# xhuan8/SoccerPlayerShapePose

Hardware: NVIDIA B200
Metric: SMPL meshes/sec fwd+bwd (higher is better)
Workload: dtype f32 (bf16x3 split on tcgen05, fp32 accumulate)

## Files before the change

### soccerplayershapepose_b200/csrc/lbs.cu

```cuda
#include "lbs_tiles.cuh"

namespace b200smpl {


struct CtaRange {
  int begin, end;
};
__device__ __forceinline__ CtaRange make_cta_range(int ngroups, int nitems) {
  const long long total = (long long)ngroups * nitems;
  CtaRange r;
  r.begin = (int)(total * blockIdx.x / gridDim.x);
  r.end = (int)(total * (blockIdx.x + 1) / gridDim.x);
  return r;
}

template <int HV>
__device__ __forceinline__ void issue_item(float4* vbuf, uint32_t* stash, uint64_t* bar, const float4* __restrict__ vp_group,
                                           const uint32_t* __restrict__ vplan, int t) {
  using SH = ItemShape<HV>;
  mbar_expect_tx(bar, SH::TX_BYTES);
  bulk_g2s(vbuf, vp_group + (size_t)t * (SH::NCH4 * 32), SH::VP_WORDS * 4, bar);
  bulk_g2s(stash, vplan + (size_t)t * SH::PLAN_WORDS, SH::PLAN_WORDS * 4, bar);
}
template <int HV>
__device__ __forceinline__ void global_to_tile_scalar(float* tile, const float* src0, size_t row_stride, int nrows,
                                                      int ncols, int lane) {
  for (int r = 0; r < 32; ++r)
    for (int c = lane; c < ItemShape<HV>::ROWS; c += 32)
      tile[r * ItemShape<HV>::HROW + c] = (r < nrows && c < ncols) ? src0[(size_t)r * row_stride + c] : 0.f;
}

constexpr int FWD_RUN = 1;
constexpr int FWD_HV = 16;
constexpr int FWD_WARPS = 8;
constexpr int FWD_THREADS = FWD_WARPS * 32;
constexpr int FWD_WARP_WORDS = ItemShape<FWD_HV>::TILE_WORDS + 2 * (ItemShape<FWD_HV>::VP_WORDS + ItemShape<FWD_HV>::PLAN_WORDS) + 4;
constexpr size_t FWD_SMEM = (size_t)(AG_WORDS + FWD_WARPS * FWD_WARP_WORDS) * 4 + 16;

template <bool HI>
__device__ __forceinline__ void load_slot2(SlotXY& s, SlotZ2& z, const float* A_s, int joint, int lane) {
  const float4* p = reinterpret_cast<const float4*>(A_s) + joint * 96 + lane;
  const float4 q0 = p[0], q1 = p[32], q2 = p[64];
  s.c0 = mk2(q0.x, q0.y); s.c1 = mk2(q0.z, q0.w); s.c2 = mk2(q1.x, q1.y); s.t = mk2(q1.z, q1.w);
  z.r20 = set_half<HI>(z.r20, q2.x); z.r21 = set_half<HI>(z.r21, q2.y);
  z.r22 = set_half<HI>(z.r22, q2.z); z.t2 = set_half<HI>(z.t2, q2.w);
}

__device__ __forceinline__ void skin_fwd4(Slots& s, const float* A_s, int lane, const uint32_t* meta_s,
                                          const float4* wts_s, uint32_t force, float tx, float ty, float tz,
                                          const float4* vp_s, float* row_out) {
  const uint4 m4 = *reinterpret_cast<const uint4*>(meta_s);
  const uint32_t mts[4] = {m4.x | force, m4.y, m4.z, m4.w};
  float4 ws[4];
#pragma unroll
  for (int i = 0; i < 4; ++i) ws[i] = wts_s[i];
  float P[12], o[12];
#pragma unroll
  for (int i = 0; i < 3; ++i) {
    const float4 v = vp_s[i * 32];
    P[i * 4] = v.x; P[i * 4 + 1] = v.y; P[i * 4 + 2] = v.z; P[i * 4 + 3] = v.w;
  }
  const f2 txy = mk2(tx, ty), tz0 = mk2(tz, 0.f);
#pragma unroll
  for (int i = 0; i < 4; ++i) {
    const uint32_t mt = mts[i];
    const float4 w = ws[i];
    if (mt & (0xFu << 20)) {
      if (mt & (1u << 20)) load_slot2<false>(s.s0, s.zA, A_s, mt & 31, lane);
      if (mt & (1u << 21)) load_slot2<true>(s.s1, s.zA, A_s, (mt >> 5) & 31, lane);
      if (mt & (1u << 22)) load_slot2<false>(s.s2, s.zB, A_s, (mt >> 10) & 31, lane);
      if (mt & (1u << 23)) load_slot2<true>(s.s3, s.zB, A_s, (mt >> 15) & 31, lane);
    }
    const f2 px = bc2(P[i * 3]), py = bc2(P[i * 3 + 1]), pz = bc2(P[i * 3 + 2]);
    f2 oxy = txy;
#define B200_SKIN_XY(sl, wk) oxy = fma2(bc2(wk), fma2(sl.c0, px, fma2(sl.c1, py, fma2(sl.c2, pz, sl.t))), oxy);
    B200_SKIN_XY(s.s0, w.x)
    B200_SKIN_XY(s.s1, w.y)
    B200_SKIN_XY(s.s2, w.z)
    B200_SKIN_XY(s.s3, w.w)
#undef B200_SKIN_XY
    f2 oz = fma2(mk2(w.x, w.y), fma2(s.zA.r20, px, fma2(s.zA.r21, py, fma2(s.zA.r22, pz, s.zA.t2))), tz0);
    oz = fma2(mk2(w.z, w.w), fma2(s.zB.r20, px, fma2(s.zB.r21, py, fma2(s.zB.r22, pz, s.zB.t2))), oz);
    o[i * 3] = lo2(oxy); o[i * 3 + 1] = hi2(oxy); o[i * 3 + 2] = lo2(oz) + hi2(oz);
  }
#pragma unroll
  for (int i = 0; i < 3; ++i)
    *reinterpret_cast<float4*>(row_out + i * 4) = make_float4(o[i * 4], o[i * 4 + 1], o[i * 4 + 2], o[i * 4 + 3]);
}

__global__ void __launch_bounds__(FWD_THREADS, 1)
lbs_fwd_kernel(const float4* __restrict__ vpB, int nc4, const float4* __restrict__ A_blk, int b0, int nb, int ngroups,
               const float* __restrict__ transl, float* __restrict__ verts, int V, int nitems, int vec_ok,
               const uint32_t* __restrict__ vplan) {
  constexpr int HV = FWD_HV;
  using SH = ItemShape<HV>;
  extern __shared__ __align__(128) float smem[];
  const int warp = threadIdx.x >> 5, lane = threadIdx.x & 31;
  float* A_s = smem;
  float* wbase = smem + AG_WORDS + warp * FWD_WARP_WORDS;
  float* tile = wbase;
  float4* vbufs = reinterpret_cast<float4*>(wbase + SH::TILE_WORDS);
  uint32_t* stash = reinterpret_cast<uint32_t*>(wbase + SH::TILE_WORDS + 2 * SH::VP_WORDS);
  uint64_t* wbar = reinterpret_cast<uint64_t*>(wbase + SH::TILE_WORDS + 2 * (SH::VP_WORDS + SH::PLAN_WORDS));
  uint64_t* bar = reinterpret_cast<uint64_t*>(smem + AG_WORDS + FWD_WARPS * FWD_WARP_WORDS);
  if (lane == 0) {
    mbar_init(&wbar[0], 1);
    mbar_init(&wbar[1], 1);
    if (warp == 0) mbar_init(bar, 1);
    asm volatile("fence.mbarrier_init.release.cluster;" ::: "memory");
  }
  __syncthreads();
  pdl_wait();
  if (threadIdx.x == 0) pdl_trigger();
  uint32_t a_phase = 0, n_used = 0;
  const CtaRange cta = make_cta_range(ngroups, nitems);
  for (int seg0 = cta.begin; seg0 < cta.end;) {
    const int g = seg0 / nitems;
    if (threadIdx.x == 0) {
      mbar_expect_tx(bar, AG_WORDS * 4);
      bulk_g2s(A_s, A_blk + (size_t)g * (AG_WORDS / 4), AG_WORDS * 4, bar);
    }
    const int seg1 = min(cta.end, (g + 1) * nitems);
    const int len = seg1 - seg0;
    const int sb = seg0 - g * nitems;
    auto off_at = [&](int n) { const int r = n / FWD_RUN; return (r * FWD_WARPS + warp) * FWD_RUN + (n - r * FWD_RUN); };
    if (off_at(0) < len) {
      const float4* vp_g = vpB + (size_t)g * nc4 * 32;
      float tx = 0.f, ty = 0.f, tz = 0.f;
      if (transl != nullptr && g * 32 + lane < nb) {
        const float* tp = transl + (size_t)(b0 + g * 32 + lane) * 3;
        tx = tp[0]; ty = tp[1]; tz = tp[2];
      }
      const int nrows = min(32, nb - g * 32);
      float* v_g = verts + (size_t)(b0 + g * 32) * V * 3;
      float* my_row = tile + lane * SH::HROW;
      if (lane == 0) {
        const uint32_t b = n_used & 1;
        issue_item<HV>(vbufs + b * (SH::NCH4 * 32), stash + b * SH::PLAN_WORDS, &wbar[b], vp_g, vplan, sb + off_at(0));
      }
      Slots sl;
      sl.zA.r20 = sl.zA.r21 = sl.zA.r22 = sl.zA.t2 = sl.zB.r20 = sl.zB.r21 = sl.zB.r22 = sl.zB.t2 = mk2(0.f, 0.f);
      mbar_wait(bar, a_phase);
      for (int n = 0;; ++n) {
        const int t = sb + off_at(n);
        if (t >= sb + len) break;
        const int tn = sb + off_at(n + 1);
        const uint32_t b = n_used & 1;
        if (tn < sb + len && lane == 0)
          issue_item<HV>(vbufs + (b ^ 1) * (SH::NCH4 * 32), stash + (b ^ 1) * SH::PLAN_WORDS, &wbar[b ^ 1], vp_g, vplan, tn);
        mbar_wait(&wbar[b], (n_used >> 1) & 1);
        const float4* vp_s = vbufs + b * (SH::NCH4 * 32) + lane;
        const uint32_t* st = stash + b * SH::PLAN_WORDS;
#pragma unroll 1
        for (int u = 0; u < HV / 4; ++u)
          skin_fwd4(sl, A_s, lane, plan_meta(st, u), plan_wts(st, u), (u == 0 && n % FWD_RUN == 0) ? (0xFu << 20) : 0u,
                    tx, ty, tz, vp_s + u * 96, my_row + u * 12);
        __syncwarp();
        {
          const int vbase = t * HV;
          const int ncols = max(0, min(HV, V - vbase)) * 3;
          float* dst0 = v_g + (size_t)vbase * 3;
          if (!vec_ok) tile_to_global_scalar<HV>(tile, dst0, (size_t)V * 3, nrows, ncols, lane);
          else tile_to_global<HV>(tile, dst0, (size_t)V * 3, nrows, ncols, lane);
        }
        __syncwarp();
        ++n_used;
      }
    }
    seg0 = seg1;
    a_phase ^= 1;
    if (seg0 < cta.end) __syncthreads();
  }
}

constexpr int BWD_HV = 8;
constexpr int BWD_WARPS = 8;
constexpr int BWD_THREADS = BWD_WARPS * 32;
constexpr int BWD_NTILE = 2;
constexpr int BWD_WARP_WORDS = BWD_NTILE * ItemShape<BWD_HV>::TILE_WORDS + 2 * (ItemShape<BWD_HV>::VP_WORDS + ItemShape<BWD_HV>::PLAN_WORDS) + 4;
constexpr size_t BWD_SMEM = (size_t)(AG_WORDS + BWD_WARPS * BWD_WARP_WORDS) * 4 + 16;

template <bool HI>
__device__ __forceinline__ void load_rot_half(SlotPair& P, const float* A_s, int joint, int lane) {
  const float4* p = reinterpret_cast<const float4*>(A_s) + joint * 96 + lane;
  const float4 q0 = p[0], q1 = p[32], q2 = p[64];
  P.R[0] = set_half<HI>(P.R[0], q0.x); P.R[3] = set_half<HI>(P.R[3], q0.y);
  P.R[1] = set_half<HI>(P.R[1], q0.z); P.R[4] = set_half<HI>(P.R[4], q0.w);
  P.R[2] = set_half<HI>(P.R[2], q1.x); P.R[5] = set_half<HI>(P.R[5], q1.y);
  P.R[6] = set_half<HI>(P.R[6], q2.x); P.R[7] = set_half<HI>(P.R[7], q2.y); P.R[8] = set_half<HI>(P.R[8], q2.z);
}

__device__ __forceinline__ void skin_bwd4(BwdState& s, const float* A_s, float* __restrict__ dA_g,
                                          int lane, const uint32_t* meta_s, const float4* wts_s, uint32_t force,
                                          const float4* vp_s, float* row_io) {
  const uint4 m4 = *reinterpret_cast<const uint4*>(meta_s);
  const uint32_t mts[4] = {m4.x | force, m4.y, m4.z, m4.w};
  float P[12], G[12];
#pragma unroll
  for (int i = 0; i < 3; ++i) {
    const float4 v = vp_s[i * 32];
    P[i * 4] = v.x; P[i * 4 + 1] = v.y; P[i * 4 + 2] = v.z; P[i * 4 + 3] = v.w;
    const float4 h = *reinterpret_cast<const float4*>(row_io + i * 4);
    G[i * 4] = h.x; G[i * 4 + 1] = h.y; G[i * 4 + 2] = h.z; G[i * 4 + 3] = h.w;
  }
  float4 w = wts_s[0];
#pragma unroll
  for (int i = 0; i < 4; ++i) {
    const uint32_t mt = mts[i];
    const float4 wn = wts_s[i < 3 ? i + 1 : 3];
    if (mt & (0xFu << 20)) {
      const uint32_t pv = s.prev;
      if (mt & (1u << 20)) { flush_half<false>(s.A, dA_g, pv & 31, lane); load_rot_half<false>(s.A, A_s, mt & 31, lane); }
      if (mt & (1u << 21)) { flush_half<true>(s.A, dA_g, (pv >> 5) & 31, lane); load_rot_half<true>(s.A, A_s, (mt >> 5) & 31, lane); }
      if (mt & (1u << 22)) { flush_half<false>(s.B, dA_g, (pv >> 10) & 31, lane); load_rot_half<false>(s.B, A_s, (mt >> 10) & 31, lane); }
      if (mt & (1u << 23)) { flush_half<true>(s.B, dA_g, (pv >> 15) & 31, lane); load_rot_half<true>(s.B, A_s, (mt >> 15) & 31, lane); }
    }
    s.prev = mt;
    const f2 px = bc2(P[i * 3]), py = bc2(P[i * 3 + 1]), pz = bc2(P[i * 3 + 2]);
    const float gx = G[i * 3], gy = G[i * 3 + 1], gz = G[i * 3 + 2];
    s.sx += gx; s.sy += gy; s.sz += gz;
    const f2 wA = mk2(w.x, w.y), wB = mk2(w.z, w.w);
    const f2 hxA = mul2(wA, bc2(gx)), hyA = mul2(wA, bc2(gy)), hzA = mul2(wA, bc2(gz));
    const f2 hxB = mul2(wB, bc2(gx)), hyB = mul2(wB, bc2(gy)), hzB = mul2(wB, bc2(gz));
    f2 qx = fma2(s.A.R[0], hxA, fma2(s.A.R[3], hyA, mul2(s.A.R[6], hzA)));
    f2 qy = fma2(s.A.R[1], hxA, fma2(s.A.R[4], hyA, mul2(s.A.R[7], hzA)));
    f2 qz = fma2(s.A.R[2], hxA, fma2(s.A.R[5], hyA, mul2(s.A.R[8], hzA)));
    qx = fma2(s.B.R[0], hxB, fma2(s.B.R[3], hyB, fma2(s.B.R[6], hzB, qx)));
    qy = fma2(s.B.R[1], hxB, fma2(s.B.R[4], hyB, fma2(s.B.R[7], hzB, qy)));
    qz = fma2(s.B.R[2], hxB, fma2(s.B.R[5], hyB, fma2(s.B.R[8], hzB, qz)));
    G[i * 3] = lo2(qx) + hi2(qx); G[i * 3 + 1] = lo2(qy) + hi2(qy); G[i * 3 + 2] = lo2(qz) + hi2(qz);
#define B200_ACC(P_, hx_, hy_, hz_)                                                                  \
  P_.D[0] = fma2(hx_, px, P_.D[0]); P_.D[1] = fma2(hx_, py, P_.D[1]); P_.D[2] = fma2(hx_, pz, P_.D[2]);   \
  P_.D[3] = add2(P_.D[3], hx_);                                                                      \
  P_.D[4] = fma2(hy_, px, P_.D[4]); P_.D[5] = fma2(hy_, py, P_.D[5]); P_.D[6] = fma2(hy_, pz, P_.D[6]);   \
  P_.D[7] = add2(P_.D[7], hy_);                                                                      \
  P_.D[8] = fma2(hz_, px, P_.D[8]); P_.D[9] = fma2(hz_, py, P_.D[9]); P_.D[10] = fma2(hz_, pz, P_.D[10]); \
  P_.D[11] = add2(P_.D[11], hz_);
    B200_ACC(s.A, hxA, hyA, hzA)
    B200_ACC(s.B, hxB, hyB, hzB)
#undef B200_ACC
    w = wn;
  }
#pragma unroll
  for (int i = 0; i < 3; ++i)
    *reinterpret_cast<float4*>(row_io + i * 4) = make_float4(G[i * 4], G[i * 4 + 1], G[i * 4 + 2], G[i * 4 + 3]);
}

__global__ void __launch_bounds__(BWD_THREADS, 1)
lbs_bwd_kernel(const float4* __restrict__ vpB, int nc4, const float4* __restrict__ A_blk, int b0, int nb, int ngroups,
               const float* __restrict__ grad_verts, int V, int nitems, int vec_ok,
               const uint32_t* __restrict__ vplan,
               __nv_bfloat16* __restrict__ dvp_hi, __nv_bfloat16* __restrict__ dvp_lo,
               float* __restrict__ dA_acc, float* __restrict__ dtr_acc) {
  constexpr int HV = BWD_HV;
  using SH = ItemShape<HV>;
  extern __shared__ __align__(128) float smem[];
  const int warp = threadIdx.x >> 5, lane = threadIdx.x & 31;
  float* A_s = smem;
  float* wbase = smem + AG_WORDS + warp * BWD_WARP_WORDS;
  float* tiles = wbase;
  float4* vbufs = reinterpret_cast<float4*>(wbase + BWD_NTILE * SH::TILE_WORDS);
  uint32_t* stash = reinterpret_cast<uint32_t*>(wbase + BWD_NTILE * SH::TILE_WORDS + 2 * SH::VP_WORDS);
  uint64_t* wbar = reinterpret_cast<uint64_t*>(wbase + BWD_NTILE * SH::TILE_WORDS + 2 * (SH::VP_WORDS + SH::PLAN_WORDS));
  uint64_t* bar = reinterpret_cast<uint64_t*>(smem + AG_WORDS + BWD_WARPS * BWD_WARP_WORDS);
  if (lane == 0) {
    mbar_init(&wbar[0], 1);
    mbar_init(&wbar[1], 1);
    if (warp == 0) mbar_init(bar, 1);
    asm volatile("fence.mbarrier_init.release.cluster;" ::: "memory");
  }
  __syncthreads();
  if (threadIdx.x == 0) pdl_trigger();
  uint32_t a_phase = 0, n_used = 0;
  const size_t row_stride = (size_t)V * 3;
  const CtaRange cta = make_cta_range(ngroups, nitems);
  for (int seg0 = cta.begin; seg0 < cta.end;) {
    const int g = seg0 / nitems;
    if (threadIdx.x == 0) {
      mbar_expect_tx(bar, AG_WORDS * 4);
      bulk_g2s(A_s, A_blk + (size_t)g * (AG_WORDS / 4), AG_WORDS * 4, bar);
    }
    const int seg1 = min(cta.end, (g + 1) * nitems);
    const int len = seg1 - seg0;
    const int it0 = seg0 - g * nitems + len * warp / BWD_WARPS;
    const int it1 = seg0 - g * nitems + len * (warp + 1) / BWD_WARPS;
    if (it0 < it1) {
      float* dA_g = dA_acc + (size_t)g * AG_WORDS;
      const float4* vp_g = vpB + (size_t)g * nc4 * 32;
      const float* dv_g = grad_verts + (size_t)(b0 + g * 32) * V * 3;
      const int nrows = max(0, min(32, nb - g * 32));
      if (lane == 0) {
        const uint32_t b = n_used & 1;
        issue_item<HV>(vbufs + b * (SH::NCH4 * 32), stash + b * SH::PLAN_WORDS, &wbar[b], vp_g, vplan, it0);
      }
      int tb = 0;
      if (vec_ok) issue_rows<HV>(tiles, dv_g + (size_t)it0 * HV * 3, row_stride, nrows, max(0, min(HV, V - it0 * HV)) * 3, lane);
      cp_async_commit();
      if (!vec_ok)
        global_to_tile_scalar<HV>(tiles, dv_g + (size_t)it0 * HV * 3, row_stride, nrows, max(0, min(HV, V - it0 * HV)) * 3, lane);
      BwdState st;
#pragma unroll
      for (int e = 0; e < AELEMS; ++e) st.A.D[e] = st.B.D[e] = mk2(0.f, 0.f);
#pragma unroll
      for (int e = 0; e < 9; ++e) st.A.R[e] = st.B.R[e] = mk2(0.f, 0.f);
      st.prev = 0u;
      st.sx = st.sy = st.sz = 0.f;
      __syncwarp();
      mbar_wait(bar, a_phase);
      for (int t = it0; t < it1; ++t) {
        const bool more = t + 1 < it1;
        const uint32_t b = n_used & 1;
        float* tile = tiles + tb * SH::TILE_WORDS;
        float* my_row = tile + lane * SH::HROW;
        if (more) {
          if (lane == 0)
            issue_item<HV>(vbufs + (b ^ 1) * (SH::NCH4 * 32), stash + (b ^ 1) * SH::PLAN_WORDS, &wbar[b ^ 1], vp_g, vplan, t + 1);
          if (vec_ok)
            issue_rows<HV>(tiles + (tb ^ 1) * SH::TILE_WORDS, dv_g + (size_t)(t + 1) * HV * 3, row_stride, nrows,
                           max(0, min(HV, V - (t + 1) * HV)) * 3, lane);
        }
        cp_async_commit();
        cp_async_wait<1>();
        __syncwarp();
        mbar_wait(&wbar[b], (n_used >> 1) & 1);
        const float4* vp_s = vbufs + b * (SH::NCH4 * 32) + lane;
        const uint32_t* ps = stash + b * SH::PLAN_WORDS;
#pragma unroll 1
        for (int u = 0; u < HV / 4; ++u)
          skin_bwd4(st, A_s, dA_g, lane, plan_meta(ps, u), plan_wts(ps, u), (u == 0 && t == it0) ? (0xFu << 20) : 0u,
                    vp_s + u * 96, my_row + u * 12);
        {
          const size_t o0 = (((size_t)(g >> 2) * (nc4 >> 1) + t * SH::NCH8) * 128 + (g & 3) * 32 + lane) * 8;
#pragma unroll
          for (int c = 0; c < SH::NCH8; ++c) {
            const float4 x = *reinterpret_cast<const float4*>(my_row + c * 8);
            const float4 y = *reinterpret_cast<const float4*>(my_row + c * 8 + 4);
            const float ch[8] = {x.x, x.y, x.z, x.w, y.x, y.y, y.z, y.w};
            store_dvp_chunk(ch, dvp_hi + o0 + c * 1024, dvp_lo ? dvp_lo + o0 + c * 1024 : nullptr);
          }
        }
        __syncwarp();
        if (more && !vec_ok)
          global_to_tile_scalar<HV>(tiles + (tb ^ 1) * SH::TILE_WORDS, dv_g + (size_t)(t + 1) * HV * 3, row_stride, nrows,
                                    max(0, min(HV, V - (t + 1) * HV)) * 3, lane);
        tb ^= 1;
        __syncwarp();
        ++n_used;
      }
      bwd_close_group(st, dA_g, dtr_acc + (size_t)g * 96, lane);
    }
    seg0 = seg1;
    a_phase ^= 1;
    if (seg0 < cta.end) __syncthreads();
  }
}

static int run_grid(int ngroups, int nitems, int warps, int num_sms) {
  const long long total = (long long)ngroups * nitems;
  return (int)std::max<long long>(1, std::min<long long>(num_sms, (total + warps - 1) / warps));
}

int launch_lbs_fwd(const DevModel& m, const float* vpB, int S, const float* A_blk, int b0, int nb,
                   const float* transl, float* verts, int num_sms, cudaStream_t st) {
  if (nb <= 0) return 0;
  const int groups = (nb + 31) / 32;
  const int nitems = m.ntiles * (TILE_V / FWD_HV);
  const int vec_ok = ((m.V & 1) == 0 && (reinterpret_cast<uintptr_t>(verts) & 7) == 0) ? 1 : 0;
  B200_SMEM_ATTR_ONCE(lbs_fwd_kernel, FWD_SMEM);
  LaunchTimer _timer("lbs_fwd", st);
  B200_CUDA_TRY(launch_k(lbs_fwd_kernel, dim3(run_grid(groups, nitems, FWD_WARPS, num_sms)), dim3(FWD_THREADS), FWD_SMEM, st, true,
                         reinterpret_cast<const float4*>(vpB), m.n_pad / 4, reinterpret_cast<const float4*>(A_blk), b0, nb, groups,
                         transl, verts, m.V, nitems, vec_ok, m.vplan));
  B200_LAUNCH_CHECK("lbs_fwd");
  return 0;
}

int launch_lbs_bwd(const DevModel& m, const float* vpB, int S, int Sw, const float* A_blk, int b0, int nb,
                   const float* grad_verts, __nv_bfloat16* dvp_hi, __nv_bfloat16* dvp_lo, float* dA_acc,
                   float* dtr_acc, int num_sms, cudaStream_t st) {
  const int groups = Sw / 32;
  const int nitems = m.ntiles * (TILE_V / BWD_HV);
  const int vec_ok = ((m.V & 1) == 0 && (reinterpret_cast<uintptr_t>(grad_verts) & 7) == 0) ? 1 : 0;
  B200_SMEM_ATTR_ONCE(lbs_bwd_kernel, BWD_SMEM);
  LaunchTimer _timer("lbs_bwd", st);
  lbs_bwd_kernel<<<run_grid(groups, nitems, BWD_WARPS, num_sms), BWD_THREADS, BWD_SMEM, st>>>(
      reinterpret_cast<const float4*>(vpB), m.n_pad / 4, reinterpret_cast<const float4*>(A_blk), b0, nb, groups, grad_verts, m.V,
      nitems, vec_ok, m.vplan, dvp_hi, dvp_lo, dA_acc, dtr_acc);
  B200_LAUNCH_CHECK("lbs_bwd");
  return 0;
}

}
```

### soccerplayershapepose_b200/csrc/lbs_tiles.cuh

```cuda
#pragma once

#include "skin_common.cuh"

namespace b200smpl {

template <int HV>
struct ItemShape {
  static constexpr int ROWS = HV * 3;
  static constexpr int HROW = ROWS + 4;
  static constexpr int TILE_WORDS = 32 * HROW;
  static constexpr int NCH4 = ROWS / 4;
  static constexpr int NCH8 = ROWS / 8;
  static constexpr int PAIRS = ROWS / 2;
  static constexpr int VP_WORDS = NCH4 * 128;
  static constexpr int PLAN_WORDS = (HV / 8) * 40;
  static constexpr uint32_t TX_BYTES = (VP_WORDS + PLAN_WORDS) * 4;
  static_assert((HROW / 4) % 2 == 1 && ROWS % 8 == 0 && HV % 8 == 0, "item shape");
};

__device__ __forceinline__ const float4* plan_wts(const uint32_t* stash, int u) {
  return reinterpret_cast<const float4*>(stash + (u >> 1) * 40 + (u & 1) * 16);
}
__device__ __forceinline__ const uint32_t* plan_meta(const uint32_t* stash, int u) {
  return stash + (u >> 1) * 40 + 32 + (u & 1) * 4;
}

template <int HV>
__device__ __forceinline__ void tile_to_global_full(const float* tile, float* dst0, size_t row_stride, int lane) {
  using SH = ItemShape<HV>;
  constexpr int RPP = 96 / SH::PAIRS, J = 32 / RPP;
  float* gp[3];
  const float* sp[3];
#pragma unroll
  for (int kk = 0; kk < 3; ++kk) {
    const int piece = kk * 32 + lane, rr = piece / SH::PAIRS, c = (piece - rr * SH::PAIRS) * 2;
    gp[kk] = dst0 + (size_t)rr * row_stride + c;
    sp[kk] = tile + rr * SH::HROW + c;
  }
  const size_t step = (size_t)RPP * row_stride;
#pragma unroll
  for (int j = 0; j < J; ++j)
#pragma unroll
    for (int kk = 0; kk < 3; ++kk) {
      st_stream2(gp[kk], *reinterpret_cast<const float2*>(sp[kk] + j * RPP * SH::HROW));
      gp[kk] += step;
    }
}
template <int HV>
__device__ __forceinline__ void tile_to_global(const float* tile, float* dst0, size_t row_stride, int nrows,
                                               int ncols, int lane) {
  using SH = ItemShape<HV>;
  if (nrows == 32 && ncols == SH::ROWS) {
    tile_to_global_full<HV>(tile, dst0, row_stride, lane);
    return;
  }
#pragma unroll 1
  for (int k = 0; k < SH::PAIRS; ++k) {
    const int piece = k * 32 + lane;
    const int r = piece / SH::PAIRS;
    const int c = (piece - r * SH::PAIRS) * 2;
    const float2 v = *reinterpret_cast<const float2*>(tile + r * SH::HROW + c);
    float* dst = dst0 + (size_t)r * row_stride + c;
    if (r < nrows) {
      if (c + 1 < ncols) st_stream2(dst, v);
      else if (c < ncols) st_stream(dst, v.x);
    }
  }
}

template <int HV>
__device__ __forceinline__ void tile_to_global_scalar(const float* tile, float* dst0, size_t row_stride, int nrows,
                                                      int ncols, int lane) {
  for (int r = 0; r < nrows; ++r)
    for (int c = lane; c < ncols; c += 32) dst0[(size_t)r * row_stride + c] = tile[r * ItemShape<HV>::HROW + c];
}

struct SlotXY {
  f2 c0, c1, c2, t;
};
struct SlotZ2 {
  f2 r20, r21, r22, t2;
};
struct Slots {
  SlotXY s0, s1, s2, s3;
  SlotZ2 zA, zB;
};

__device__ __forceinline__ void cp_async8_zfill(void* dst_smem, const void* src, int src_bytes) {
  asm volatile("cp.async.ca.shared.global.L2::256B [%0], [%1], 8, %2;" ::"r"(smem_addr(dst_smem)), "l"(src), "r"(src_bytes)
               : "memory");
}
__device__ __forceinline__ void cp_async_commit() { asm volatile("cp.async.commit_group;" ::: "memory"); }
template <int N>
__device__ __forceinline__ void cp_async_wait() { asm volatile("cp.async.wait_group %0;" ::"n"(N) : "memory"); }
template <int HV>
__device__ __forceinline__ void issue_rows(float* tile, const float* __restrict__ src0, size_t row_stride, int nrows,
                                           int ncols, int lane) {
  using SH = ItemShape<HV>;
  constexpr int RPP = 96 / SH::PAIRS, J = 32 / RPP;
  if (nrows == 32 && ncols == SH::ROWS) {
    const float* gp[3];
    float* sp[3];
#pragma unroll
    for (int kk = 0; kk < 3; ++kk) {
      const int piece = kk * 32 + lane, rr = piece / SH::PAIRS, c = (piece - rr * SH::PAIRS) * 2;
      gp[kk] = src0 + (size_t)rr * row_stride + c;
      sp[kk] = tile + rr * SH::HROW + c;
    }
    const size_t step = (size_t)RPP * row_stride;
#pragma unroll
    for (int j = 0; j < J; ++j)
#pragma unroll
      for (int kk = 0; kk < 3; ++kk) {
        cp_async8_zfill(sp[kk] + j * RPP * SH::HROW, gp[kk], 8);
        gp[kk] += step;
      }
    return;
  }
#pragma unroll 1
  for (int k = 0; k < SH::PAIRS; ++k) {
    const int piece = k * 32 + lane;
    const int r = piece / SH::PAIRS;
    const int c = (piece - r * SH::PAIRS) * 2;
    const bool ok = r < nrows && c < ncols;
    const int bytes = ok ? (c + 1 < ncols ? 8 : 4) : 0;
    cp_async8_zfill(tile + r * SH::HROW + c, ok ? src0 + (size_t)r * row_stride + c : src0, bytes);
  }
}

struct SlotPair {
  f2 R[9];
  f2 D[AELEMS];
};
struct BwdState {
  SlotPair A, B;
  uint32_t prev;
  float sx, sy, sz;
};
template <bool HI>
__device__ __forceinline__ void flush_half(SlotPair& P, float* dA_g, int joint, int lane) {
  float* p = dA_g + (size_t)joint * AELEMS * 32 + lane;
#pragma unroll
  for (int e = 0; e < AELEMS; ++e) {
    red_add(p + e * 32, get_half<HI>(P.D[e]));
    P.D[e] = set_half<HI>(P.D[e], 0.f);
  }
}

__device__ __forceinline__ void bwd_close_group(BwdState& s, float* dA_g, float* dtr_g, int lane) {
  flush_half<false>(s.A, dA_g, s.prev & 31, lane);
  flush_half<true>(s.A, dA_g, (s.prev >> 5) & 31, lane);
  flush_half<false>(s.B, dA_g, (s.prev >> 10) & 31, lane);
  flush_half<true>(s.B, dA_g, (s.prev >> 15) & 31, lane);
  red_add(dtr_g + lane, s.sx);
  red_add(dtr_g + 32 + lane, s.sy);
  red_add(dtr_g + 64 + lane, s.sz);
  s.sx = s.sy = s.sz = 0.f;
}


}
```

Baseline: 6.948 million.

## Pipeline backward skinning loads in three stages with cp.async mbarrier completion

The backward LBS kernel goes from a double-buffered scheme, which used separate cp.async commit/wait groups and bulk-copy mbarriers, to a three-stage ring. Each stage's mbarrier tracks both the bulk vertex and plan copies and the per-lane 16-byte cp.async gradient-row copies via cp.async.mbarrier.arrive. Gradient rows are now fetched as aligned 16-byte chunks regardless of alignment, and each lane reads at a per-row phase offset, so the scalar fallback path and the vec_ok flag are removed. The intent is deeper prefetch and fewer warp syncs and wait stalls. The costs are more shared memory per warp and over-fetching at row boundaries.

Measured after the change: 6.325 million, median of 6. -9.0%, worse.

```diff
diff --git a/soccerplayershapepose_b200/csrc/lbs.cu b/soccerplayershapepose_b200/csrc/lbs.cu
--- a/soccerplayershapepose_b200/csrc/lbs.cu
+++ b/soccerplayershapepose_b200/csrc/lbs.cu
@@ -21,13 +21,6 @@
   mbar_expect_tx(bar, SH::TX_BYTES);
   bulk_g2s(vbuf, vp_group + (size_t)t * (SH::NCH4 * 32), SH::VP_WORDS * 4, bar);
   bulk_g2s(stash, vplan + (size_t)t * SH::PLAN_WORDS, SH::PLAN_WORDS * 4, bar);
-}
-template <int HV>
-__device__ __forceinline__ void global_to_tile_scalar(float* tile, const float* src0, size_t row_stride, int nrows,
-                                                      int ncols, int lane) {
-  for (int r = 0; r < 32; ++r)
-    for (int c = lane; c < ItemShape<HV>::ROWS; c += 32)
-      tile[r * ItemShape<HV>::HROW + c] = (r < nrows && c < ncols) ? src0[(size_t)r * row_stride + c] : 0.f;
 }
 
 constexpr int FWD_RUN = 1;
@@ -176,9 +169,41 @@
 constexpr int BWD_HV = 8;
 constexpr int BWD_WARPS = 8;
 constexpr int BWD_THREADS = BWD_WARPS * 32;
-constexpr int BWD_NTILE = 2;
-constexpr int BWD_WARP_WORDS = BWD_NTILE * ItemShape<BWD_HV>::TILE_WORDS + 2 * (ItemShape<BWD_HV>::VP_WORDS + ItemShape<BWD_HV>::PLAN_WORDS) + 4;
+constexpr int BWD_STAGES = 3;
+constexpr int BWD_STAGE_WORDS = ItemShape<BWD_HV>::TILE_WORDS + ItemShape<BWD_HV>::VP_WORDS + ItemShape<BWD_HV>::PLAN_WORDS;
+constexpr int BWD_BAR_WORDS = (2 * BWD_STAGES + 3) / 4 * 4;
+constexpr int BWD_WARP_WORDS = BWD_STAGES * BWD_STAGE_WORDS + BWD_BAR_WORDS;
 constexpr size_t BWD_SMEM = (size_t)(AG_WORDS + BWD_WARPS * BWD_WARP_WORDS) * 4 + 16;
+static_assert(BWD_SMEM <= 227 * 1024, "lbs_bwd shared memory");
+static_assert(BWD_STAGE_WORDS % 4 == 0 && BWD_WARP_WORDS % 4 == 0, "16-byte aligned staging buffers");
+
+template <int HV>
+__device__ __forceinline__ void issue_bwd_item(float* tile, float4* vbuf, uint32_t* stash, uint64_t* bar,
+                                               const float4* __restrict__ vp_group, const uint32_t* __restrict__ vplan,
+                                               const float* dv_g, size_t row_stride, int nrows, int ncols, int t,
+                                               int lane) {
+  using SH = ItemShape<HV>;
+  constexpr int GR = SH::HROW / 4;
+  if (lane == 0) {
+    mbar_expect_tx(bar, SH::TX_BYTES);
+    bulk_g2s(vbuf, vp_group + (size_t)t * (SH::NCH4 * 32), SH::VP_WORDS * 4, bar);
+    bulk_g2s(stash, vplan + (size_t)t * SH::PLAN_WORDS, SH::PLAN_WORDS * 4, bar);
+  }
+  if (ncols > 0) {
+#pragma unroll
+    for (int k = 0; k < GR; ++k) {
+      const int piece = k * 32 + lane, r = piece / GR, q = piece - r * GR;
+      if (r < nrows) {
+        const uintptr_t a = reinterpret_cast<uintptr_t>(dv_g + (size_t)r * row_stride + (size_t)t * SH::ROWS);
+        const uintptr_t w0 = a & ~(uintptr_t)15;
+        if (w0 + 16 * q < a + (uintptr_t)ncols * 4)
+          asm volatile("cp.async.cg.shared.global [%0], [%1], 16;" ::"r"(smem_addr(tile + r * SH::HROW + 4 * q)),
+                       "l"(w0 + 16 * q) : "memory");
+      }
+    }
+  }
+  asm volatile("cp.async.mbarrier.arrive.noinc.shared::cta.b64 [%0];" ::"r"(smem_addr(bar)) : "memory");
+}
 
 template <bool HI>
 __device__ __forceinline__ void load_rot_half(SlotPair& P, const float* A_s, int joint, int lane) {
@@ -192,7 +217,7 @@
 
 __device__ __forceinline__ void skin_bwd4(BwdState& s, const float* A_s, float* __restrict__ dA_g,
                                           int lane, const uint32_t* meta_s, const float4* wts_s, uint32_t force,
-                                          const float4* vp_s, float* row_io) {
+                                          const float4* vp_s, const float* row_in, float* row_out) {
   const uint4 m4 = *reinterpret_cast<const uint4*>(meta_s);
   const uint32_t mts[4] = {m4.x | force, m4.y, m4.z, m4.w};
   float P[12], G[12];
@@ -200,9 +225,9 @@
   for (int i = 0; i < 3; ++i) {
     const float4 v = vp_s[i * 32];
     P[i * 4] = v.x; P[i * 4 + 1] = v.y; P[i * 4 + 2] = v.z; P[i * 4 + 3] = v.w;
-    const float4 h = *reinterpret_cast<const float4*>(row_io + i * 4);
-    G[i * 4] = h.x; G[i * 4 + 1] = h.y; G[i * 4 + 2] = h.z; G[i * 4 + 3] = h.w;
-  }
+  }
+#pragma unroll
+  for (int i = 0; i < 12; ++i) G[i] = row_in[i];
   float4 w = wts_s[0];
 #pragma unroll
   for (int i = 0; i < 4; ++i) {
@@ -243,12 +268,12 @@
   }
 #pragma unroll
   for (int i = 0; i < 3; ++i)
-    *reinterpret_cast<float4*>(row_io + i * 4) = make_float4(G[i * 4], G[i * 4 + 1], G[i * 4 + 2], G[i * 4 + 3]);
+    *reinterpret_cast<float4*>(row_out + i * 4) = make_float4(G[i * 4], G[i * 4 + 1], G[i * 4 + 2], G[i * 4 + 3]);
 }
 
 __global__ void __launch_bounds__(BWD_THREADS, 1)
 lbs_bwd_kernel(const float4* __restrict__ vpB, int nc4, const float4* __restrict__ A_blk, int b0, int nb, int ngroups,
-               const float* __restrict__ grad_verts, int V, int nitems, int vec_ok,
+               const float* __restrict__ grad_verts, int V, int nitems,
                const uint32_t* __restrict__ vplan,
                __nv_bfloat16* __restrict__ dvp_hi, __nv_bfloat16* __restrict__ dvp_lo,
                float* __restrict__ dA_acc, float* __restrict__ dtr_acc) {
@@ -259,13 +284,13 @@
   float* A_s = smem;
   float* wbase = smem + AG_WORDS + warp * BWD_WARP_WORDS;
   float* tiles = wbase;
-  float4* vbufs = reinterpret_cast<float4*>(wbase + BWD_NTILE * SH::TILE_WORDS);
-  uint32_t* stash = reinterpret_cast<uint32_t*>(wbase + BWD_NTILE * SH::TILE_WORDS + 2 * SH::VP_WORDS);
-  uint64_t* wbar = reinterpret_cast<uint64_t*>(wbase + BWD_NTILE * SH::TILE_WORDS + 2 * (SH::VP_WORDS + SH::PLAN_WORDS));
+  float4* vbufs = reinterpret_cast<float4*>(wbase + BWD_STAGES * SH::TILE_WORDS);
+  uint32_t* stash = reinterpret_cast<uint32_t*>(wbase + BWD_STAGES * (SH::TILE_WORDS + SH::VP_WORDS));
+  uint64_t* wbar = reinterpret_cast<uint64_t*>(wbase + BWD_STAGES * BWD_STAGE_WORDS);
   uint64_t* bar = reinterpret_cast<uint64_t*>(smem + AG_WORDS + BWD_WARPS * BWD_WARP_WORDS);
   if (lane == 0) {
-    mbar_init(&wbar[0], 1);
-    mbar_init(&wbar[1], 1);
+#pragma unroll
+    for (int k = 0; k < BWD_STAGES; ++k) mbar_init(&wbar[k], 33);
     if (warp == 0) mbar_init(bar, 1);
     asm volatile("fence.mbarrier_init.release.cluster;" ::: "memory");
   }
@@ -287,17 +312,18 @@
     if (it0 < it1) {
       float* dA_g = dA_acc + (size_t)g * AG_WORDS;
       const float4* vp_g = vpB + (size_t)g * nc4 * 32;
-      const float* dv_g = grad_verts + (size_t)(b0 + g * 32) * V * 3;
+      const float* dv_g = grad_verts + (size_t)(b0 + g * 32) * row_stride;
       const int nrows = max(0, min(32, nb - g * 32));
-      if (lane == 0) {
-        const uint32_t b = n_used & 1;
-        issue_item<HV>(vbufs + b * (SH::NCH4 * 32), stash + b * SH::PLAN_WORDS, &wbar[b], vp_g, vplan, it0);
-      }
-      int tb = 0;
-      if (vec_ok) issue_rows<HV>(tiles, dv_g + (size_t)it0 * HV * 3, row_stride, nrows, max(0, min(HV, V - it0 * HV)) * 3, lane);
-      cp_async_commit();
-      if (!vec_ok)
-        global_to_tile_scalar<HV>(tiles, dv_g + (size_t)it0 * HV * 3, row_stride, nrows, max(0, min(HV, V - it0 * HV)) * 3, lane);
+      const float* my_dv = lane < nrows ? dv_g + (size_t)lane * row_stride : nullptr;
+      const int ph = (int)((reinterpret_cast<uintptr_t>(my_dv) >> 2) & 3);
+      auto ncols_of = [&](int t) { return max(0, min(HV, V - t * HV)) * 3; };
+      auto issue = [&](int t, uint32_t k) {
+        issue_bwd_item<HV>(tiles + k * SH::TILE_WORDS, vbufs + k * (SH::NCH4 * 32), stash + k * SH::PLAN_WORDS, &wbar[k],
+                           vp_g, vplan, dv_g, row_stride, nrows, ncols_of(t), t, lane);
+      };
+#pragma unroll
+      for (int k = 0; k < BWD_STAGES - 1; ++k)
+        if (it0 + k < it1) issue(it0 + k, (n_used + k) % BWD_STAGES);
       BwdState st;
 #pragma unroll
       for (int e = 0; e < AELEMS; ++e) st.A.D[e] = st.B.D[e] = mk2(0.f, 0.f);
@@ -305,30 +331,19 @@
       for (int e = 0; e < 9; ++e) st.A.R[e] = st.B.R[e] = mk2(0.f, 0.f);
       st.prev = 0u;
       st.sx = st.sy = st.sz = 0.f;
-      __syncwarp();
       mbar_wait(bar, a_phase);
       for (int t = it0; t < it1; ++t) {
-        const bool more = t + 1 < it1;
-        const uint32_t b = n_used & 1;
-        float* tile = tiles + tb * SH::TILE_WORDS;
-        float* my_row = tile + lane * SH::HROW;
-        if (more) {
-          if (lane == 0)
-            issue_item<HV>(vbufs + (b ^ 1) * (SH::NCH4 * 32), stash + (b ^ 1) * SH::PLAN_WORDS, &wbar[b ^ 1], vp_g, vplan, t + 1);
-          if (vec_ok)
-            issue_rows<HV>(tiles + (tb ^ 1) * SH::TILE_WORDS, dv_g + (size_t)(t + 1) * HV * 3, row_stride, nrows,
-                           max(0, min(HV, V - (t + 1) * HV)) * 3, lane);
-        }
-        cp_async_commit();
-        cp_async_wait<1>();
-        __syncwarp();
-        mbar_wait(&wbar[b], (n_used >> 1) & 1);
-        const float4* vp_s = vbufs + b * (SH::NCH4 * 32) + lane;
-        const uint32_t* ps = stash + b * SH::PLAN_WORDS;
+        const uint32_t k = n_used % BWD_STAGES;
+        if (t + BWD_STAGES - 1 < it1) issue(t + BWD_STAGES - 1, (n_used + BWD_STAGES - 1) % BWD_STAGES);
+        float* my_row = tiles + k * SH::TILE_WORDS + lane * SH::HROW;
+        mbar_wait(&wbar[k], (n_used / BWD_STAGES) & 1);
+        for (int c = my_dv != nullptr ? ncols_of(t) : 0; c < SH::ROWS; ++c) my_row[ph + c] = 0.f;
+        const float4* vp_s = vbufs + k * (SH::NCH4 * 32) + lane;
+        const uint32_t* ps = stash + k * SH::PLAN_WORDS;
 #pragma unroll 1
         for (int u = 0; u < HV / 4; ++u)
           skin_bwd4(st, A_s, dA_g, lane, plan_meta(ps, u), plan_wts(ps, u), (u == 0 && t == it0) ? (0xFu << 20) : 0u,
-                    vp_s + u * 96, my_row + u * 12);
+                    vp_s + u * 96, my_row + ph + u * 12, my_row + u * 12);
         {
           const size_t o0 = (((size_t)(g >> 2) * (nc4 >> 1) + t * SH::NCH8) * 128 + (g & 3) * 32 + lane) * 8;
 #pragma unroll
@@ -339,11 +354,6 @@
             store_dvp_chunk(ch, dvp_hi + o0 + c * 1024, dvp_lo ? dvp_lo + o0 + c * 1024 : nullptr);
           }
         }
-        __syncwarp();
-        if (more && !vec_ok)
-          global_to_tile_scalar<HV>(tiles + (tb ^ 1) * SH::TILE_WORDS, dv_g + (size_t)(t + 1) * HV * 3, row_stride, nrows,
-                                    max(0, min(HV, V - (t + 1) * HV)) * 3, lane);
-        tb ^= 1;
         __syncwarp();
         ++n_used;
       }
@@ -380,12 +390,11 @@
                    float* dtr_acc, int num_sms, cudaStream_t st) {
   const int groups = Sw / 32;
   const int nitems = m.ntiles * (TILE_V / BWD_HV);
-  const int vec_ok = ((m.V & 1) == 0 && (reinterpret_cast<uintptr_t>(grad_verts) & 7) == 0) ? 1 : 0;
   B200_SMEM_ATTR_ONCE(lbs_bwd_kernel, BWD_SMEM);
   LaunchTimer _timer("lbs_bwd", st);
   lbs_bwd_kernel<<<run_grid(groups, nitems, BWD_WARPS, num_sms), BWD_THREADS, BWD_SMEM, st>>>(
       reinterpret_cast<const float4*>(vpB), m.n_pad / 4, reinterpret_cast<const float4*>(A_blk), b0, nb, groups, grad_verts, m.V,
-      nitems, vec_ok, m.vplan, dvp_hi, dvp_lo, dA_acc, dtr_acc);
+      nitems, m.vplan, dvp_hi, dvp_lo, dA_acc, dtr_acc);
   B200_LAUNCH_CHECK("lbs_bwd");
   return 0;
 }
diff --git a/soccerplayershapepose_b200/csrc/lbs_tiles.cuh b/soccerplayershapepose_b200/csrc/lbs_tiles.cuh
--- a/soccerplayershapepose_b200/csrc/lbs_tiles.cuh
+++ b/soccerplayershapepose_b200/csrc/lbs_tiles.cuh
@@ -86,48 +86,6 @@
   SlotZ2 zA, zB;
 };
 
-__device__ __forceinline__ void cp_async8_zfill(void* dst_smem, const void* src, int src_bytes) {
-  asm volatile("cp.async.ca.shared.global.L2::256B [%0], [%1], 8, %2;" ::"r"(smem_addr(dst_smem)), "l"(src), "r"(src_bytes)
-               : "memory");
-}
-__device__ __forceinline__ void cp_async_commit() { asm volatile("cp.async.commit_group;" ::: "memory"); }
-template <int N>
-__device__ __forceinline__ void cp_async_wait() { asm volatile("cp.async.wait_group %0;" ::"n"(N) : "memory"); }
-template <int HV>
-__device__ __forceinline__ void issue_rows(float* tile, const float* __restrict__ src0, size_t row_stride, int nrows,
-                                           int ncols, int lane) {
-  using SH = ItemShape<HV>;
-  constexpr int RPP = 96 / SH::PAIRS, J = 32 / RPP;
-  if (nrows == 32 && ncols == SH::ROWS) {
-    const float* gp[3];
-    float* sp[3];
-#pragma unroll
-    for (int kk = 0; kk < 3; ++kk) {
-      const int piece = kk * 32 + lane, rr = piece / SH::PAIRS, c = (piece - rr * SH::PAIRS) * 2;
-      gp[kk] = src0 + (size_t)rr * row_stride + c;
-      sp[kk] = tile + rr * SH::HROW + c;
-    }
-    const size_t step = (size_t)RPP * row_stride;
-#pragma unroll
-    for (int j = 0; j < J; ++j)
-#pragma unroll
-      for (int kk = 0; kk < 3; ++kk) {
-        cp_async8_zfill(sp[kk] + j * RPP * SH::HROW, gp[kk], 8);
-        gp[kk] += step;
-      }
-    return;
-  }
-#pragma unroll 1
-  for (int k = 0; k < SH::PAIRS; ++k) {
-    const int piece = k * 32 + lane;
-    const int r = piece / SH::PAIRS;
-    const int c = (piece - r * SH::PAIRS) * 2;
-    const bool ok = r < nrows && c < ncols;
-    const int bytes = ok ? (c + 1 < ncols ? 8 : 4) : 0;
-    cp_async8_zfill(tile + r * SH::HROW + c, ok ? src0 + (size_t)r * row_stride + c : src0, bytes);
-  }
-}
-
 struct SlotPair {
   f2 R[9];
   f2 D[AELEMS];
```
